# afanasyev-ilya/VectorGraphLibrary

Measured on AMD Instinct MI355X. Metric: TEPS (edges/s) BFS + SSSP on RMAT-24; value = direction-optimising BFS, sssp_value_teps = direction-optimising Bellman-Ford, higher is better.
Workload: dtype int32; 1 GPU; BFS direction-optimising on RMAT scale-24 (edge factor 32), 1xMI355X; vertices=16777216, edges=536870912, seed=1, parallelism=edge-cut x1, exchange_transport=none, vertex_numbering=degree-sorted (total)

## Files before the change

profiles/microbench/bfs_ab.py:

```python
#!/usr/bin/env python3
import argparse
import os
import sys
import time

sys.path.insert(0, os.path.dirname(os.path.dirname(os.path.dirname(os.path.abspath(__file__)))))
import torch

import bench
from vectorgraphlibrary_amd import api

ap = argparse.ArgumentParser()
ap.add_argument("--scale", type=int, default=24)
ap.add_argument("--steps", type=int, default=32)
ap.add_argument("--warmup", type=int, default=4)
ap.add_argument("--rounds", type=int, default=2)
ap.add_argument("--per-source", action="store_true")
ap.add_argument("variants", nargs="+")
args = ap.parse_args()

ctx = api.Context(0)
V = 1 << args.scale
src, dst = ctx.gen_rmat(args.scale, 32, 1)
g = api.Graph.from_coo(ctx, V, src, dst, with_incoming=True, renumber="total")
E = g.E
del src, dst
handles = {None: g}


def handle_for(heads):
    if heads not in handles:
        os.environ["VGL_BFS_HEADS"] = heads
        handles[heads] = api.Graph(ctx, V, g.out_rowptr, g.out_adj, g.in_rowptr, g.in_adj)
        print(f"handle for VGL_BFS_HEADS={heads}: {handles[heads].info()}", flush=True)
    return handles[heads]


sources = bench.pick_sources(g.out_rowptr, args.steps + args.warmup, 1)
ref = {}
for s in sources:
    lv, _ = api.bfs(g, s, api.BFS_TOP_DOWN, raw=True)
    ref[s] = lv.clone()
KERNELS = ("bfs_bottom_up", "bfs_bottom_up_heavy", "bfs_top_down", "bfs_small_levels", "bfs_bitmap_expand", "gnf")
variants = []
for v in args.variants:
    name, _, kv = v.partition(":")
    variants.append((name, dict(x.split("=", 1) for x in kv.split(",") if x)))
touched = set(k for _, env in variants for k in env)
results = {name: [] for name, _ in variants}
for rnd in range(args.rounds):
    for name, env in variants:
        for k in touched:
            os.environ.pop(k, None)
        os.environ.update(env)
        g = handle_for(env.get("VGL_BFS_HEADS"))
        bad = 0
        for s in sources[:args.warmup]:
            api.bfs(g, s, api.BFS_DIRECTION_OPT, raw=True)
        torch.cuda.synchronize()
        t0 = time.perf_counter()
        for s in sources[args.warmup:]:
            api.bfs(g, s, api.BFS_DIRECTION_OPT, raw=True)
        torch.cuda.synchronize()
        ms = (time.perf_counter() - t0) / args.steps * 1e3
        ctx.timing(True)
        stats = []
        prev = {k: 0.0 for k in KERNELS}
        for s in sources[args.warmup:]:
            lv, st = api.bfs(g, s, api.BFS_DIRECTION_OPT, raw=True)
            stats.append(st)
            bad += int(api.count_not_equal(ctx, lv, ref[s]) != 0)
            if args.per_source and rnd == 0:
                now = {k: ctx.timing_get(k)[1] for k in KERNELS}
                print(f"    {name} source {s}: td/bu {st['td_steps']}/{st['bu_steps']} td_edges {st['td_edges']} bu_probes {st['bu_edges']} bu_found {st['bu_found']} | "
                      + " ".join(f"{k.replace('bfs_', '')} {(now[k] - prev[k]) * 1e3:.0f}" for k in KERNELS if now[k] > prev[k]) + " us")
                prev = now
        torch.cuda.synchronize()
        kern = {k: ctx.timing_get(k) for k in KERNELS}
        ctx.timing(False)
# ... 6 lines not shown
```

vectorgraphlibrary_amd/csrc/bfs.hip:

```cpp
#include "vgl_hip_internal.h"
#include <chrono>
#include "vgl_gnf.h"
#include "vgl_blocked.h"

#ifndef VGL_BU_HEAVY_LANES
#define VGL_BU_HEAVY_LANES 16
#endif

__global__ __launch_bounds__(VGL_BLOCK) void vgl_k_bfs_init(int32_t V, int32_t source, int32_t *levels)
{
    for (int32_t v = blockIdx.x * VGL_BLOCK + threadIdx.x; v < V; v += gridDim.x * VGL_BLOCK)
        levels[v] = (v == source) ? 1 : -1;
}

__global__ __launch_bounds__(VGL_BLOCK) void vgl_k_bfs_init_all(int32_t fill, int32_t source, int32_t prev, int32_t *levels, int64_t words, uint64_t *visited,
                                                                uint64_t *front, uint64_t *next, uint32_t *tickets, unsigned long long *list_count)
{
    if (blockIdx.x == 0 && threadIdx.x == 0) {
        *list_count = 0ULL;
        if (prev >= fill) levels[prev] = -1;
        if (source >= fill) levels[source] = 1;
    }
    for (int32_t v = blockIdx.x * VGL_BLOCK + threadIdx.x; v < fill; v += gridDim.x * VGL_BLOCK)
        levels[v] = (v == source) ? 1 : -1;
    for (int64_t w = (int64_t)blockIdx.x * VGL_BLOCK + threadIdx.x; w < words; w += (int64_t)gridDim.x * VGL_BLOCK) {
        const uint64_t bit = (w == (source >> 6)) ? (1ULL << (source & 63)) : 0ULL;
        visited[w] = bit; front[w] = bit; next[w] = 0;
    }
    if (blockIdx.x == 0)
        for (int i = threadIdx.x; i < 4 * VGL_TICKET_WORDS; i += VGL_BLOCK) tickets[i] = 0;
}

__global__ __launch_bounds__(VGL_BLOCK) void vgl_k_tile_first(int32_t F, const int64_t *offs, int32_t *tile_first)
{
    for (int32_t p = blockIdx.x * VGL_BLOCK + threadIdx.x; p < F; p += gridDim.x * VGL_BLOCK) {
        const int64_t t0 = (offs[p] + VGL_TILE - 1) / VGL_TILE;
        const int64_t t1 = (offs[p + 1] + VGL_TILE - 1) / VGL_TILE;
        for (int64_t t = t0; t < t1; t++) tile_first[t] = p;
        if (offs[p] < offs[p + 1] && offs[p + 1] == offs[F]) tile_first[(offs[F] + VGL_TILE - 1) / VGL_TILE] = p;
    }
}

template <bool EMIT, bool COUNT, bool FILTER = true>
__global__ __launch_bounds__(VGL_BLOCK) void vgl_k_td_expand(const int32_t *ids, const int64_t *offs, const int32_t *tile_first,
                                                             int32_t F, int64_t M, const int64_t *rowptr, const int32_t *adj,
                                                             int32_t row_base, const uint64_t *visited, int32_t *levels,
                                                             int32_t next_level, uint64_t *next, int64_t *partials, uint32_t *ticket, int64_t *counters)
{
    __shared__ int s_map[VGL_TILE];
    __shared__ int64_t s_base[VGL_TILE];
    __shared__ int s_w[VGL_WAVES];
    const int64_t e0 = (int64_t)blockIdx.x * VGL_TILE;
    const int n = (int)min((int64_t)VGL_TILE, M - e0);
    const int p_first = tile_first[blockIdx.x];
    const int p_last = tile_first[blockIdx.x + 1];
    const int np = p_last - p_first + 1;
    const bool staged = np <= VGL_TILE;
    if (staged)
        for (int k = threadIdx.x; k < np; k += VGL_BLOCK) {
            const int p = p_first + k;
            s_base[k] = rowptr[ids[p] - row_base] - offs[p];
        }
// ... 22 lines not shown
#pragma unroll
        for (int j = 0; j < VGL_EPT; j++) unvis[j] = dsts[j] >= 0 && !((vw[j] >> (dsts[j] & 63)) & 1ULL);
    } else {
#pragma unroll
        for (int j = 0; j < VGL_EPT; j++) unvis[j] = dsts[j] >= 0;
    }
#else
#pragma unroll
    for (int j = 0; j < VGL_EPT; j++) unvis[j] = dsts[j] >= 0 && (!FILTER || !((visited[dsts[j] >> 6] >> (dsts[j] & 63)) & 1ULL));
#endif
#if VGL_TD_BATCH & 2
    int32_t lv[VGL_EPT];
#pragma unroll
    for (int j = 0; j < VGL_EPT; j++) lv[j] = levels[unvis[j] ? dsts[j] : 0];
#pragma unroll
    for (int j = 0; j < VGL_EPT; j++) fresh[j] = unvis[j] && lv[j] == -1;
#else
#pragma unroll
    for (int j = 0; j < VGL_EPT; j++) fresh[j] = unvis[j] && levels[dsts[j]] == -1;
#endif
    if (!COUNT) {
#pragma unroll
        for (int j = 0; j < VGL_EPT; j++)
            if (fresh[j]) {
                levels[dsts[j]] = next_level;
                if (EMIT) atomicOr((unsigned long long *)&next[dsts[j] >> 6], 1ULL << (dsts[j] & 63));
            }
        return;
    }
    __shared__ int64_t s64[VGL_WAVES];
    unsigned long long old[VGL_EPT];
#pragma unroll
    for (int j = 0; j < VGL_EPT; j++) {
        old[j] = ~0ULL;
// ... 206 lines not shown
        cpre += vgl_load_agent(vt_cnt + t);
        dpre += vgl_load_agent(vt_deg + t);
    }
    if (threadIdx.x == 0) {
        offs[ctot] = dtot;
        host[C_SKIPPED] = 0;
        vgl_publish2(counters, host, seq, C_FRONT, (int64_t)ctot, C_NEIGH, dtot);
    }
}
constexpr int VGL_SCAN_BLOCKS = 1024;
__device__ inline uint32_t vgl_match8(const int4 a, const int4 c, int32_t value)
{
    return (a.x == value) | ((a.y == value) << 1) | ((a.z == value) << 2) | ((a.w == value) << 3) |
           ((c.x == value) << 4) | ((c.y == value) << 5) | ((c.z == value) << 6) | ((c.w == value) << 7);
}
__global__ __launch_bounds__(VGL_BLOCK) void vgl_k_bfs_scan_bound(int32_t nrows, int32_t ntiles, int32_t row_base, const int32_t *levels, int32_t level,
                                                                 const int32_t *vt_min_deg, uint8_t *front_bytes, uint8_t *visited_bytes,
                                                                 int64_t *partials, uint32_t *ticket, int64_t *counters,
                                                                 volatile int64_t *host, int64_t seq, int32_t stale_front)
{
    __shared__ int64_t s64[VGL_WAVES];
    if (stale_front >= 0 && blockIdx.x == 0 && threadIdx.x == 0) front_bytes[stale_front >> 3] = 0;
    int64_t f = 0, m = 0;
    const int32_t stride = (int32_t)gridDim.x;
    int32_t t = (int32_t)blockIdx.x;
    for (; t + stride < ntiles && (t + stride + 1) * VGL_TILE <= nrows; t += 2 * stride) {
        const int32_t va = row_base + t * VGL_TILE + (int32_t)threadIdx.x * VGL_EPT, vb = va + stride * VGL_TILE;
        const int4 a0 = *reinterpret_cast<const int4 *>(levels + va), a1 = *reinterpret_cast<const int4 *>(levels + va + 4);
        const int4 b0 = *reinterpret_cast<const int4 *>(levels + vb), b1 = *reinterpret_cast<const int4 *>(levels + vb + 4);
        const uint32_t fa = vgl_match8(a0, a1, level), fb = vgl_match8(b0, b1, level);
        front_bytes[va >> 3] = (uint8_t)fa; visited_bytes[va >> 3] = (uint8_t)(0xFFu ^ vgl_match8(a0, a1, -1));
        front_bytes[vb >> 3] = (uint8_t)fb; visited_bytes[vb >> 3] = (uint8_t)(0xFFu ^ vgl_match8(b0, b1, -1));
        f += __popc(fa) + __popc(fb);
        m += (int64_t)__popc(fa) * vt_min_deg[t] + (int64_t)__popc(fb) * vt_min_deg[t + stride];
    }
    for (; t < ntiles; t += stride) {
        const int32_t r0 = t * VGL_TILE + (int32_t)threadIdx.x * VGL_EPT;
        if (r0 >= nrows) continue;
        const int32_t v0 = row_base + r0;
        uint32_t aux;
        const vgl_pred_equal_i32 pred{levels, level};
        const uint32_t bits = pred.bits8(v0, min(VGL_EPT, nrows - r0), &aux);
        front_bytes[v0 >> 3] = (uint8_t)bits;
        visited_bytes[v0 >> 3] = (uint8_t)aux;
        f += __popc(bits);
        m += (int64_t)__popc(bits) * vt_min_deg[t];
    }
    f = vgl_block_reduce_add(f, s64);
    m = vgl_block_reduce_add(m, s64);
    uint32_t dep = 0;
    if (threadIdx.x == 0) dep = vgl_put_agent(partials + 2 * blockIdx.x, f) ^ vgl_put_agent(partials + 2 * blockIdx.x + 1, m);
    if (!vgl_last_block(ticket, dep)) return;
    f = 0; m = 0;
    for (int b = threadIdx.x; b < (int)gridDim.x; b += VGL_BLOCK) { f += vgl_load_agent(partials + 2 * b); m += vgl_load_agent(partials + 2 * b + 1); }
    f = vgl_block_reduce_add(f, s64);
    m = vgl_block_reduce_add(m, s64);
// ... 622 lines not shown
    if (threadIdx.x == 0) { partials[blockIdx.x * 2] = cnt; partials[blockIdx.x * 2 + 1] = deg; }
}
__global__ __launch_bounds__(VGL_BLOCK) void vgl_k_apply_fold(int n, const int64_t *partials, int64_t *counters)
{
    __shared__ int64_t s64[VGL_WAVES];
    int64_t a = 0, b = 0;
    for (int i = threadIdx.x; i < n; i += VGL_BLOCK) { a += partials[i * 2]; b += partials[i * 2 + 1]; }
    a = vgl_block_reduce_add(a, s64);
    b = vgl_block_reduce_add(b, s64);
    if (threadIdx.x == 0) { counters[C_TMP0] = a; counters[C_TMP1] = b; }
}


template <bool EMIT, bool COUNT>
static void vgl_td_expand_launch(vgl_hip_ctx *c, vgl_hip_graph *g, int32_t F, int64_t M, const uint64_t *visited, int32_t *levels,
                                 int32_t next_level, uint64_t *next, bool filter = true)
{
    const auto kernel = filter ? vgl_k_td_expand<EMIT, COUNT, true> : vgl_k_td_expand<EMIT, COUNT, false>;
    hipLaunchKernelGGL(kernel, dim3((unsigned)vgl_ceil_div(M, VGL_TILE)), dim3(VGL_BLOCK), 0, c->stream, g->ids, g->offs, g->tile_first, F, M,
                       g->out.rowptr, g->out.adj, g->row_begin, visited, levels, next_level, next, COUNT ? g->bu_partials : (int64_t *)nullptr,
                       COUNT ? g->tickets + 3 * VGL_TICKET_WORDS : (uint32_t *)nullptr, COUNT ? c->d_counters : (int64_t *)nullptr);
}

constexpr int64_t VGL_TD_COUNT_TILES = 8192;
static int vgl_bfs_td_launch(vgl_hip_ctx *c, vgl_hip_graph *g, int32_t F, int64_t M, int32_t *levels, int32_t next_level, bool emit,
                             bool have_tile_first, bool count = false, bool filter = true)
{
    if (F <= 0 || M <= 0) return 0;
    if (!have_tile_first) hipLaunchKernelGGL(vgl_k_tile_first, dim3(vgl_grid(F, VGL_BLOCK, 8192)), dim3(VGL_BLOCK), 0, c->stream, F, g->offs, g->tile_first);
    {
        vgl_timed_launch tl(c, "bfs_top_down");
        if (emit && count) vgl_td_expand_launch<true, true>(c, g, F, M, g->bm_visited, levels, next_level, g->bm_next, filter);
        else if (emit) vgl_td_expand_launch<true, false>(c, g, F, M, g->bm_visited, levels, next_level, g->bm_next, filter);
        else vgl_td_expand_launch<false, false>(c, g, F, M, g->bm_visited, levels, next_level, g->bm_next, filter);
    }
    VGL_HIP_TRY(hipGetLastError());
    return 0;
}

int vgl_bfs_bm_gnf(vgl_hip_ctx *c, vgl_hip_graph *g, const uint64_t *front, bool count, bool write, int64_t M_known, bool advance, const vgl_do_hint *hint)
{
    const vgl_do_hint no_hint = {0, 0, 0, 0};
    const int64_t word0 = g->row_begin >> 6;
    const int64_t nwords = vgl_ceil_div(g->row_end, 64) - word0;
    const unsigned nb = (unsigned)vgl_ceil_div(nwords, VGL_BLOCK);
    if (count) {
        const int64_t seq = vgl_next_seq(c);
        {
            vgl_timed_launch tl(c, "gnf");
// ... 140 lines not shown

struct vgl_bfs_traversal {
    vgl_hip_ctx *c;
    vgl_hip_graph *g;
    int mode;
    int32_t *levels;
    vgl_bfs_params p;
    int32_t V;
    int64_t E, words, factor;
    unsigned bm_blocks;
    unsigned long long *list_count;
    std::chrono::steady_clock::time_point t0;

    int32_t source = -1;
    int32_t cur = 1;
    vgl_bfs_front front = vgl_bfs_front::bitmap;
    bool bottom_up = false;
    bool hint_ready = false, skipped = false, finished = false;
    int64_t F = 0, M = 0, prevF = 0, visited_total = 0;
    vgl_hip_bfs_stats st = {0, 0, 0, 0, 0, 0, 0, 0, 0, 0, 0};

    vgl_bfs_traversal(vgl_hip_ctx *c_, vgl_hip_graph *g_, int mode_, int32_t *levels_)
        : c(c_), g(g_), mode(mode_), levels(levels_), p(vgl_bfs_params_of(c_->bfs, g_->V, mode_)), V(g_->V), E(g_->out.edges)
    {
        words = vgl_ceil_div(V, 64);
        factor = vgl_do_factor(E, V);
        bm_blocks = (unsigned)vgl_ceil_div(words, VGL_BLOCK);
        list_count = reinterpret_cast<unsigned long long *>(c->d_counters + C_HEAVY);
    }

// ... 21 lines not shown
        const char *done = "count done (bitmap)";
        if (front != vgl_bfs_front::levels) {
            const bool advance = front == vgl_bfs_front::pending;
            const vgl_do_hint hint = {prevF, visited_total, (int64_t)V, factor};
            const bool hinted = hint_ready && advance && p.use_hints;
            VGL_TRY(vgl_bfs_bm_gnf(c, g, g->bm_front, true, false, -1, advance, hinted ? &hint : nullptr));
            skipped = hinted && c->h_counters[C_SKIPPED] != 0;
            front = skipped ? vgl_bfs_front::bitmap : vgl_bfs_front::counted_bitmap;
        } else if (p.scan_bound && g->nvtiles <= 8192) {
            const int64_t seq = vgl_next_seq(c);
            const int64_t scan_tiles = std::max<int64_t>(1, std::min<int64_t>(g->nvtiles, vgl_ceil_div(g->reach_rows, VGL_TILE)));
            const int32_t scan_rows = (int32_t)std::min<int64_t>(g->nrows, scan_tiles * VGL_TILE);
            {
                vgl_timed_launch tl(c, "gnf");
                hipLaunchKernelGGL(vgl_k_bfs_scan_bound, dim3((unsigned)std::min<int64_t>(scan_tiles, VGL_SCAN_BLOCKS)), dim3(VGL_BLOCK), 0, c->stream, scan_rows,
                                   (int32_t)scan_tiles, g->row_begin, (const int32_t *)levels, cur, (const int32_t *)g->vt_min_deg, (uint8_t *)g->bm_front.p,
                                   (uint8_t *)g->bm_visited.p, g->bu_partials, g->tickets + 0 * VGL_TICKET_WORDS, c->d_counters,
                                   (volatile int64_t *)c->h_counters, seq, source >= scan_rows ? source : -1);
            }
            VGL_HIP_TRY(hipGetLastError());
            VGL_TRY(vgl_wait_counters(c, seq));
            front = vgl_bfs_front::bitmap;
            const int64_t f = c->h_counters[C_FRONT], m_lb = c->h_counters[C_NEIGH];
            if (vgl_do_turn_bottom_up(f, m_lb, prevF, visited_total + f, V, factor)) {
                F = f; M = m_lb; skipped = true; hint_ready = false;
                trace("count done (levels scan)");
                return 0;
            }
            VGL_TRY(vgl_bfs_bm_gnf(c, g, g->bm_front, true, false, -1, false, nullptr));
            front = vgl_bfs_front::counted_bitmap;
        } else {
            vgl_pred_equal_i32 pred{levels, cur};
            VGL_TRY(vgl_gnf_run(c, g, pred, g->ids, g->offs, (uint8_t *)g->bm_front.p, (uint8_t *)g->bm_visited.p, nullptr, false, true));
            front = vgl_bfs_front::counted_scan;
            done = "count done (levels scan)";
        }
        F = c->h_counters[C_FRONT]; M = c->h_counters[C_NEIGH];
        hint_ready = false;
        trace(done);
        return 0;
    }

    int small_levels(int32_t listF, int32_t src, bool from_bitmap)
    {
        if (from_bitmap) {
            vgl_timed_launch tl(c, "bfs_bitmap_expand");
            hipLaunchKernelGGL(vgl_k_bm_expand, dim3(bm_blocks), dim3(VGL_BLOCK), 0, c->stream, words, g->bm_front, g->out.rowptr, g->out.adj, g->bm_visited,
                               g->bm_next, levels, cur + 1, g->ids, list_count, (int32_t)VGL_SMALL_F, g->bu_partials);
        }
        const int64_t seq = vgl_next_seq(c);
        {
            vgl_timed_launch tl(c, "bfs_small_levels");
            hipLaunchKernelGGL(vgl_k_bfs_small_levels, dim3(1), dim3(VGL_SMALL_THREADS), 0, c->stream, g->ids, listF, src, g->out.rowptr, g->out.adj,
                               g->bm_visited, g->bm_next, levels, from_bitmap ? cur + 1 : cur, p.small_m, c->d_counters, (volatile int64_t *)c->h_counters,
                               seq, from_bitmap ? list_count : (unsigned long long *)nullptr, (const int64_t *)g->bu_partials, from_bitmap ? (int)bm_blocks : 0,
                               g->bm_front, g->offs, g->tile_first);
        }
        VGL_HIP_TRY(hipGetLastError());
        VGL_TRY(vgl_wait_counters(c, seq));
        return 0;
    }
    void book_small(int64_t firstF)
    {
        const int64_t *h = c->h_counters;
        const int64_t run = h[C_TMP0], later = h[C_TMP1];
        st.td_steps += (int32_t)run; st.edges_examined += h[C_EDGES]; st.td_edges += h[C_EDGES];
        st.td_frontier += firstF + later;
        visited_total += later; st.levels += (int32_t)(run - 1); st.frontier_total += later;
        if (run > 1) prevF = h[C_JUMP];
// ... 10 lines not shown
        const int64_t m_level = c->h_counters[C_CHANGED], n_next = c->h_counters[C_BU_FOUND];
        book_top_down(F, m_level);
        prevF = F;
        cur++;
        if (n_next == 0) { finished = true; return 0; }
        if (c->h_counters[C_TMP0] > 0) {
            begin_level(n_next);
            prevF = n_next;
            book_small(n_next);
        } else front = vgl_bfs_front::pending;
        return 0;
    }
    int blocked_level()
    {
        trace("counted -> blocked level");
        VGL_TRY(vgl_bfs_blocked_level(c, g, levels, cur + 1));
        trace("blocked level done");
        front = vgl_bfs_front::pending;
        book_top_down(F, M);
        cur++;
        return 0;
    }
    int top_down_level()
    {
        switch (front) {
        case vgl_bfs_front::ids: break;
        case vgl_bfs_front::counted_bitmap: VGL_TRY(vgl_bfs_bm_gnf(c, g, g->bm_front, false, true, M)); break;
        case vgl_bfs_front::counted_scan: {
            vgl_pred_equal_i32 pred{levels, cur};
            vgl_timed_launch tl(c, "gnf");
            hipLaunchKernelGGL(vgl_k_gnf_write<vgl_pred_equal_i32>, dim3((unsigned)g->nvtiles), dim3(VGL_BLOCK), 0, c->stream, pred,
                               g->nrows, g->row_begin, g->out.rowptr, g->vt_cnt_off, g->vt_deg_off, g->ids, g->offs, (int32_t *)nullptr, (int64_t)0);
            break;
        }
        default: VGL_FAIL("bfs_run: internal error (frontier not counted)");
        }
        trace("ids written");
        const bool have_tile_first = front != vgl_bfs_front::counted_scan;
        if (p.small_m > 0 && have_tile_first && F <= VGL_SMALL_F && M <= p.small_m) {
            trace("counted + ids -> list kernel");
            VGL_TRY(small_levels((int32_t)F, -1, false));
            trace("list kernel done");
            book_small(F);
            return 0;
        }
        const bool is_late = late();
        const bool emit = M <= p.td_emit_edges || is_late;
        const bool td_counts = emit && p.use_hints && vgl_ceil_div(M, VGL_TILE) <= VGL_TD_COUNT_TILES;
        const bool filter = is_late || (double)visited_total >= p.td_filter_share * (double)V;
        trace(emit ? "counted + ids -> top-down (emitting)" : "counted + ids -> top-down (levels only)");
        VGL_TRY(vgl_bfs_td_launch(c, g, (int32_t)F, M, levels, cur + 1, emit, have_tile_first, td_counts, filter));
        trace("top-down done");
        hint_ready = td_counts && F > 0 && M > 0;
        front = emit ? vgl_bfs_front::pending : vgl_bfs_front::levels;
        book_top_down(F, M);
        cur++;
        return 0;
    }
    int bottom_up_level()
    {
        if (front == vgl_bfs_front::levels || front == vgl_bfs_front::pending) VGL_FAIL("bfs_run: internal error (bitmaps missing)");
        int64_t seq = 0;
        trace("-> bottom-up");
        const bool filtered = F <= p.filter_f;
        if (filtered) trace("bottom-up through the folded frontier");
        VGL_TRY(vgl_bfs_bu_launch(c, g, levels, cur + 1, g->bm_visited, g->bm_front, g->bm_next, &seq, filtered));
        hipLaunchKernelGGL(vgl_k_bm_advance, dim3(vgl_grid(words, VGL_BLOCK, 8192)), dim3(VGL_BLOCK), 0, c->stream, words, g->bm_visited, g->bm_front, g->bm_next);
        VGL_HIP_TRY(hipGetLastError());
        VGL_TRY(vgl_wait_counters(c, seq));
        st.bu_steps++; st.edges_examined += c->h_counters[C_BU_EDGES];
        st.bu_edges += c->h_counters[C_BU_EDGES]; st.bu_found += c->h_counters[C_BU_FOUND];
        F = c->h_counters[C_BU_FOUND]; M = 0;
        front = vgl_bfs_front::bitmap;
        cur++;
        return 0;
    }

    int run(int32_t source_, int32_t prev = -1)
    {
        source = source_;
        const int32_t fill = prev >= 0 ? g->reach_rows : V;
        hipLaunchKernelGGL(vgl_k_bfs_init_all, dim3(vgl_grid(std::max<int64_t>(fill, words), VGL_BLOCK, 8192)), dim3(VGL_BLOCK), 0, c->stream, fill, source, prev,
                           levels, words, g->bm_visited, g->bm_front, g->bm_next, g->tickets, list_count);
        t0 = std::chrono::steady_clock::now();
        if (p.small_m > 0) {
            VGL_TRY(small_levels(1, source, false));
            if (c->h_counters[C_TMP0] > 0) {
                begin_level(1);
                prevF = 1;
                book_small(1);
            }
        }
        while (!finished) {
            if (front != vgl_bfs_front::ids && !bottom_up) VGL_TRY(count());
            if (F == 0) break;
            begin_level(F);
            if (mode == VGL_HIP_BFS_DIRECTION_OPT) {
                if (!bottom_up) bottom_up = vgl_do_turn_bottom_up(F, M, prevF, visited_total, V, factor);
// ... 35 lines not shown
    spec.gather_rows = 1;
    spec.skip_self = 1;
    spec.value_bits = 1;
    return vgl_blocked_build(c, g->out, g->nrows, g->row_begin, g->V, spec, &g->blk_bfs);
}

int vgl_hip_bfs_init(vgl_hip_ctx *c, int32_t V, int32_t source, int32_t *d_levels)
{
    if (!c || !d_levels) VGL_FAIL("bfs_init: null argument");
    if (source < 0 || source >= V) VGL_FAIL("bfs_init: source vertex out of range");
    hipLaunchKernelGGL(vgl_k_bfs_init, dim3(vgl_grid(V, VGL_BLOCK, 8192)), dim3(VGL_BLOCK), 0, c->stream, V, source, d_levels);
    VGL_HIP_TRY(hipGetLastError());
    return 0;
}

static int vgl_bfs_run_from(vgl_hip_ctx *c, vgl_hip_graph *g, int32_t source, int32_t prev, int mode, int32_t *d_levels, vgl_hip_bfs_stats *stats)
{
    if (!c || !g || !d_levels) VGL_FAIL("bfs_run: null argument");
    if (g->row_begin != 0 || g->row_end != g->V) VGL_FAIL("bfs_run: graph handle must own all rows (use the step API for shards)");
    if (mode != VGL_HIP_BFS_TOP_DOWN && mode != VGL_HIP_BFS_DIRECTION_OPT) VGL_FAIL("bfs_run: unknown mode");
    if (mode == VGL_HIP_BFS_DIRECTION_OPT && !g->in.rowptr) VGL_FAIL("bfs_run: direction-optimising mode needs the incoming CSR");
    if (source < 0 || source >= g->V) VGL_FAIL("bfs_run: source vertex out of range");
    vgl_ctx_refresh_env(c);
    vgl_bfs_traversal t(c, g, mode, d_levels);
    VGL_TRY(t.run(source, prev));
    if (stats) *stats = t.st;
    return 0;
}

int vgl_hip_bfs_run(vgl_hip_ctx *c, vgl_hip_graph *g, int32_t source, int mode, int32_t *d_levels, vgl_hip_bfs_stats *stats)
{
    return vgl_bfs_run_from(c, g, source, -1, mode, d_levels, stats);
}

int vgl_hip_bfs_run_batch(vgl_hip_ctx *c, vgl_hip_graph *g, const int32_t *sources, int32_t count, int mode, int32_t *d_levels, vgl_hip_bfs_stats *stats)
{
    if (!sources || count < 0) VGL_FAIL("bfs_run_batch: null argument");
    for (int32_t i = 0; i < count; i++)
        VGL_TRY(vgl_bfs_run_from(c, g, sources[i], i > 0 ? sources[i - 1] : -1, mode, d_levels, stats ? stats + i : nullptr));
    return 0;
}

int vgl_hip_bfs_step_top_down(vgl_hip_ctx *c, vgl_hip_graph *g, int32_t *d_levels, int32_t level, const uint64_t *d_visited_bits,
                              int64_t *local_frontier, int64_t *local_edges)
{
    if (!c || !g || !d_levels) VGL_FAIL("bfs_step_top_down: null argument");
    const uint64_t *visited = d_visited_bits;
    if (!visited) {
        hipLaunchKernelGGL(vgl_k_levels_to_bitmap<true>, dim3(vgl_grid(g->V, VGL_BLOCK, 8192)), dim3(VGL_BLOCK), 0, c->stream, g->V, d_levels, -1,
                           g->bm_visited);
        visited = g->bm_visited;
    }
    vgl_pred_equal_i32 pred{d_levels, level};
    VGL_TRY(vgl_gnf_run(c, g, pred, g->ids, g->offs, nullptr, nullptr, nullptr, true, true));
    const int64_t F = c->h_counters[C_FRONT], M = c->h_counters[C_NEIGH];
    if (local_frontier) *local_frontier = F;
    if (local_edges) *local_edges = M;
    if (F > 0 && M > 0) {
        hipLaunchKernelGGL(vgl_k_tile_first, dim3(vgl_grid(F, VGL_BLOCK, 8192)), dim3(VGL_BLOCK), 0, c->stream, (int32_t)F, g->offs, g->tile_first);
        vgl_timed_launch tl(c, "bfs_top_down");
        vgl_td_expand_launch<false, false>(c, g, (int32_t)F, M, visited, d_levels, level + 1, nullptr);
    }
    VGL_HIP_TRY(hipGetLastError());
    return 0;
}

int vgl_hip_bfs_step_top_down_bits(vgl_hip_ctx *c, vgl_hip_graph *g, int32_t *d_levels, int32_t level, const uint64_t *d_visited_bits,
                                   const uint64_t *d_front_bits, uint64_t *d_next_bits, int64_t *local_frontier, int64_t *local_edges)
{
    if (!c || !g || !d_levels || !d_visited_bits || !d_front_bits || !d_next_bits) VGL_FAIL("bfs_step_top_down_bits: null argument");
    if (g->row_begin & 63) VGL_FAIL("bfs_step_top_down_bits: the first owned row must be a multiple of 64");
    VGL_TRY(vgl_bfs_bm_gnf(c, g, d_front_bits, true, true));
    const int64_t F = c->h_counters[C_FRONT], M = c->h_counters[C_NEIGH];
    if (local_frontier) *local_frontier = F;
    if (local_edges) *local_edges = M;
    const int64_t emit_edges = c->bfs.shard_td_emit_edges >= 0 ? c->bfs.shard_td_emit_edges : vgl_bfs_td_emit_edges(g->V);
    const bool emit = M <= emit_edges;
    const int64_t words = vgl_ceil_div(g->V, 64);
    if (emit) VGL_TRY(vgl_zero_words(c, d_next_bits, words));
    if (F > 0 && M > 0) {
        vgl_timed_launch tl(c, "bfs_top_down");
        if (emit) vgl_td_expand_launch<true, false>(c, g, (int32_t)F, M, d_visited_bits, d_levels, level + 1, d_next_bits);
        else vgl_td_expand_launch<false, false>(c, g, (int32_t)F, M, d_visited_bits, d_levels, level + 1, d_next_bits);
    }
    if (!emit) {
        vgl_timed_launch tl(c, "gnf");
        hipLaunchKernelGGL(vgl_k_levels_to_bitmap<false>, dim3(vgl_grid(g->V, VGL_BLOCK, 8192)), dim3(VGL_BLOCK), 0, c->stream, g->V, (const int32_t *)d_levels, level + 1, d_next_bits);
    }
    VGL_HIP_TRY(hipGetLastError());
    return 0;
}

int vgl_hip_bfs_step_bottom_up(vgl_hip_ctx *c, vgl_hip_graph *g, int32_t *d_levels, int32_t level, const uint64_t *d_visited_bits,
                               const uint64_t *d_front_bits, uint64_t *d_next_bits, int64_t *found, int64_t *probed)
{
    if (!c || !g || !d_levels || !d_visited_bits || !d_front_bits || !d_next_bits) VGL_FAIL("bfs_step_bottom_up: null argument");
    if (!g->in.rowptr) VGL_FAIL("bfs_step_bottom_up: the incoming CSR of the owned rows is required");
    VGL_TRY(vgl_zero_words(c, d_next_bits, vgl_ceil_div(g->V, 64)));
// ... 105 lines not shown
```

vectorgraphlibrary_amd/csrc/context.hip:

```cpp
#include "vgl_hip_internal.h"
#include <unordered_set>
#include <cstdio>
#include <cstring>
#include <mutex>
#include <algorithm>

static thread_local std::string g_last_error;

int vgl_set_error(const char *file, int line, const char *msg)
{
    char buf[512];
    const char *base = strrchr(file, '/');
    snprintf(buf, sizeof(buf), "vgl_hip: %s (%s:%d)", msg, base ? base + 1 : file, line);
    g_last_error = buf;
    return 1;
}

static hipMemPool_t g_lib_pool[64];
static bool g_lib_pool_tried[64];
static std::mutex g_lib_pool_mutex;
hipMemPool_t vgl_lib_pool(int device)
{
    if (device < 0 || device >= 64) return nullptr;
    std::lock_guard<std::mutex> lock(g_lib_pool_mutex);
// ... 43 lines not shown
        for (char **e = environ; *e; e++)
            if (strncmp(*e, "VGL_", 4) == 0)
                if (const char *eq = strchr(*e, '=')) c->env[std::string(*e, (size_t)(eq - *e))] = std::string(eq + 1);
    vgl_bfs_tunables t;
    auto str = [&](const char *n) -> const char * { auto it = c->env.find(n); return it == c->env.end() ? nullptr : it->second.c_str(); };
    auto on = [&](const char *n) { const char *v = str(n); return v && v[0] == '1'; };
    if (const char *v = str("VGL_TD_EMIT_EDGES")) t.td_emit_edges = atoll(v);
    if (const char *v = str("VGL_BFS_SMALL_M")) t.small_m = atoll(v);
    if (const char *v = str("VGL_BFS_BM_EXPAND")) t.bm_expand = atoll(v);
    if (const char *v = str("VGL_BFS_FILTER_F")) t.filter_f = atoll(v);
    if (const char *v = str("VGL_SHARD_TD_EMIT_EDGES")) t.shard_td_emit_edges = atoll(v);
    if (const char *v = str("VGL_TD_FILTER_SHARE")) t.td_filter_share = atof(v);
    if (const char *v = str("VGL_TD_LATE_SHARE")) t.td_late_share = atof(v);
    if (const char *v = str("VGL_BFS_BLOCKED_SHARE")) t.blocked_share = atof(v);
    if (const char *v = str("VGL_SHARD_SPARSE_CAP")) t.shard_sparse_cap = std::max(0, atoi(v));
    t.no_hint = on("VGL_BFS_NO_HINT"); t.no_scan_bound = on("VGL_BFS_NO_SCAN_BOUND"); t.trace = on("VGL_BFS_TRACE");
    c->bfs = t;
}
const char *vgl_env(vgl_hip_ctx *c, const char *name)
{
    vgl_ctx_refresh_env(c);
    auto it = c->env.find(name);
    return it == c->env.end() ? nullptr : it->second.c_str();
}
int64_t vgl_env_int(vgl_hip_ctx *c, const char *name, int64_t dflt, int64_t lo, int64_t hi)
{
    const char *s = vgl_env(c, name);
    const int64_t v = (s && *s) ? strtoll(s, nullptr, 10) : dflt;
    return std::min(hi, std::max(lo, v));
}

// ... 243 lines not shown
```

vectorgraphlibrary_amd/csrc/vgl_gnf.h:

```cpp
#pragma once
#include "vgl_hip_internal.h"

#ifdef __HIPCC__

struct vgl_pred_equal_i32 {
    const int32_t *values; int32_t value;
    __device__ uint32_t bits8(int32_t v0, int nvalid, uint32_t *aux) const
    {
        uint32_t b = 0, n = 0;
        if (nvalid == 8) {
            const int4 a = *reinterpret_cast<const int4 *>(values + v0);
            const int4 c = *reinterpret_cast<const int4 *>(values + v0 + 4);
            b = (a.x == value) | ((a.y == value) << 1) | ((a.z == value) << 2) | ((a.w == value) << 3) |
                ((c.x == value) << 4) | ((c.y == value) << 5) | ((c.z == value) << 6) | ((c.w == value) << 7);
            n = (a.x != -1) | ((a.y != -1) << 1) | ((a.z != -1) << 2) | ((a.w != -1) << 3) |
                ((c.x != -1) << 4) | ((c.y != -1) << 5) | ((c.z != -1) << 6) | ((c.w != -1) << 7);
        } else {
            for (int j = 0; j < nvalid; j++) {
                const int32_t x = values[v0 + j];
                b |= (uint32_t)(x == value) << j;
                n |= (uint32_t)(x != -1) << j;
            }
        }
        *aux = n;
        return b;
    }
};
struct vgl_pred_nonzero_i32 {
    const int32_t *flags;
    __device__ uint32_t bits8(int32_t v0, int nvalid, uint32_t *aux) const
    {
        uint32_t b = 0;
        *aux = 0;
        if (nvalid == 8) {
            const int4 a = *reinterpret_cast<const int4 *>(flags + v0);
            const int4 c = *reinterpret_cast<const int4 *>(flags + v0 + 4);
            b = (a.x != 0) | ((a.y != 0) << 1) | ((a.z != 0) << 2) | ((a.w != 0) << 3) |
                ((c.x != 0) << 4) | ((c.y != 0) << 5) | ((c.z != 0) << 6) | ((c.w != 0) << 7);
        } else {
            for (int j = 0; j < nvalid; j++) b |= (uint32_t)(flags[v0 + j] != 0) << j;
        }
        return b;
// ... 272 lines not shown
```

vectorgraphlibrary_amd/csrc/vgl_hip_internal.h:

```cpp
#pragma once
#include <hip/hip_runtime.h>
#include <stdint.h>
#include <string>
#include <map>
#include <memory>
#include <vector>
#include "../../include/vgl_hip.h"

constexpr int VGL_BLOCK = 256;
constexpr int VGL_EPT = 8;
constexpr int VGL_TILE = VGL_BLOCK * VGL_EPT;
constexpr int VGL_WAVES = VGL_BLOCK / 64;
constexpr int VGL_FOLD_WORDS = 2048;

int vgl_set_error(const char *file, int line, const char *msg);
#define VGL_FAIL(msg) return vgl_set_error(__FILE__, __LINE__, (msg))
#define VGL_HIP_TRY(expr)                                                          \
    do {                                                                           \
        hipError_t _e = (expr);                                                    \
        if (_e != hipSuccess) return vgl_set_error(__FILE__, __LINE__, hipGetErrorString(_e)); \
    } while (0)
#define VGL_TRY(expr)            \
    do {                         \
        int _s = (expr);         \
// ... 8 lines not shown
    C_NSLOTS = 32
};
constexpr int VGL_NSHARD = 1024;

struct vgl_timing_slot {
    int64_t launches = 0;
    std::vector<std::pair<hipEvent_t, hipEvent_t>> pending;
    double total_ms = 0.0;
};

struct vgl_bfs_tunables {
    int64_t td_emit_edges = -1, small_m = -1, bm_expand = -1, shard_td_emit_edges = -1, filter_f = -1;
    double td_filter_share = -1.0, td_late_share = -1.0, blocked_share = -1.0;
    int shard_sparse_cap = -1;
    bool no_hint = false, no_scan_bound = false, trace = false;
};

struct vgl_hip_ctx {
    std::map<std::string, std::string> env;
    uint64_t env_signature = 0;
    vgl_bfs_tunables bfs;
    int device = 0;
    hipStream_t stream = nullptr;
    bool own_stream = false;
    int64_t *d_counters = nullptr;
    int64_t *d_shards = nullptr;
    int64_t *h_counters = nullptr;
    int64_t publish_seq = 0;
    double *d_partials = nullptr;
    size_t partials_cap = 0;
// ... 410 lines not shown
```

Before: 1933 billion edges/s.

## Use per-traversal level offsets in batched BFS to skip level-array refills

Batched BFS no longer clears the levels array between sources. Each traversal writes levels shifted by a running offset, and every kernel treats values at or below the offset floor as unvisited: top-down expand, the scan-bound count, the new level predicate and the init kernel. A full refill still runs on the first and last source, or when the offset nears INT32 overflow. This removes most per-source O(reach_rows) init traffic, at the cost of an extra compare parameter threaded through many kernels and intermediate level arrays that are not directly meaningful.

```diff
diff --git a/profiles/microbench/bfs_ab.py b/profiles/microbench/bfs_ab.py
--- a/profiles/microbench/bfs_ab.py
+++ b/profiles/microbench/bfs_ab.py
@@ -16,6 +16,7 @@
 ap.add_argument("--warmup", type=int, default=4)
 ap.add_argument("--rounds", type=int, default=2)
 ap.add_argument("--per-source", action="store_true")
+ap.add_argument("--batch", action="store_true")
 ap.add_argument("variants", nargs="+")
 args = ap.parse_args()
 
@@ -41,6 +42,7 @@
 for s in sources:
     lv, _ = api.bfs(g, s, api.BFS_TOP_DOWN, raw=True)
     ref[s] = lv.clone()
+lv_buf = ctx.empty(V, torch.int32)
 KERNELS = ("bfs_bottom_up", "bfs_bottom_up_heavy", "bfs_top_down", "bfs_small_levels", "bfs_bitmap_expand", "gnf")
 variants = []
 for v in args.variants:
@@ -59,10 +61,15 @@
             api.bfs(g, s, api.BFS_DIRECTION_OPT, raw=True)
         torch.cuda.synchronize()
         t0 = time.perf_counter()
-        for s in sources[args.warmup:]:
-            api.bfs(g, s, api.BFS_DIRECTION_OPT, raw=True)
+        if args.batch:
+            lv_batch, _ = api.bfs_batch(g, sources[args.warmup:], api.BFS_DIRECTION_OPT, levels=lv_buf)
+        else:
+            for s in sources[args.warmup:]:
+                api.bfs(g, s, api.BFS_DIRECTION_OPT, raw=True)
         torch.cuda.synchronize()
         ms = (time.perf_counter() - t0) / args.steps * 1e3
+        if args.batch:
+            bad += int(api.count_not_equal(ctx, lv_batch, ref[sources[-1]]) != 0)
         ctx.timing(True)
         stats = []
         prev = {k: 0.0 for k in KERNELS}
diff --git a/vectorgraphlibrary_amd/csrc/bfs.hip b/vectorgraphlibrary_amd/csrc/bfs.hip
--- a/vectorgraphlibrary_amd/csrc/bfs.hip
+++ b/vectorgraphlibrary_amd/csrc/bfs.hip
@@ -13,16 +13,17 @@
         levels[v] = (v == source) ? 1 : -1;
 }
 
-__global__ __launch_bounds__(VGL_BLOCK) void vgl_k_bfs_init_all(int32_t fill, int32_t source, int32_t prev, int32_t *levels, int64_t words, uint64_t *visited,
-                                                                uint64_t *front, uint64_t *next, uint32_t *tickets, unsigned long long *list_count)
+__global__ __launch_bounds__(VGL_BLOCK) void vgl_k_bfs_init_all(int32_t fill, int32_t source, int32_t first, int32_t reset, int32_t *levels, int64_t words,
+                                                                uint64_t *visited, uint64_t *front, uint64_t *next, uint32_t *tickets,
+                                                                unsigned long long *list_count)
 {
     if (blockIdx.x == 0 && threadIdx.x == 0) {
         *list_count = 0ULL;
-        if (prev >= fill) levels[prev] = -1;
-        if (source >= fill) levels[source] = 1;
+        if (reset >= fill) levels[reset] = -1;
+        if (source >= fill) levels[source] = first;
     }
     for (int32_t v = blockIdx.x * VGL_BLOCK + threadIdx.x; v < fill; v += gridDim.x * VGL_BLOCK)
-        levels[v] = (v == source) ? 1 : -1;
+        levels[v] = (v == source) ? first : -1;
     for (int64_t w = (int64_t)blockIdx.x * VGL_BLOCK + threadIdx.x; w < words; w += (int64_t)gridDim.x * VGL_BLOCK) {
         const uint64_t bit = (w == (source >> 6)) ? (1ULL << (source & 63)) : 0ULL;
         visited[w] = bit; front[w] = bit; next[w] = 0;
@@ -45,7 +46,8 @@
 __global__ __launch_bounds__(VGL_BLOCK) void vgl_k_td_expand(const int32_t *ids, const int64_t *offs, const int32_t *tile_first,
                                                              int32_t F, int64_t M, const int64_t *rowptr, const int32_t *adj,
                                                              int32_t row_base, const uint64_t *visited, int32_t *levels,
-                                                             int32_t next_level, uint64_t *next, int64_t *partials, uint32_t *ticket, int64_t *counters)
+                                                             int32_t next_level, int32_t floor, uint64_t *next, int64_t *partials, uint32_t *ticket,
+                                                             int64_t *counters)
 {
     __shared__ int s_map[VGL_TILE];
     __shared__ int64_t s_base[VGL_TILE];
@@ -98,10 +100,10 @@
 #pragma unroll
     for (int j = 0; j < VGL_EPT; j++) lv[j] = levels[unvis[j] ? dsts[j] : 0];
 #pragma unroll
-    for (int j = 0; j < VGL_EPT; j++) fresh[j] = unvis[j] && lv[j] == -1;
+    for (int j = 0; j < VGL_EPT; j++) fresh[j] = unvis[j] && lv[j] <= floor;
 #else
 #pragma unroll
-    for (int j = 0; j < VGL_EPT; j++) fresh[j] = unvis[j] && levels[dsts[j]] == -1;
+    for (int j = 0; j < VGL_EPT; j++) fresh[j] = unvis[j] && levels[dsts[j]] <= floor;
 #endif
     if (!COUNT) {
 #pragma unroll
@@ -338,10 +340,15 @@
     return (a.x == value) | ((a.y == value) << 1) | ((a.z == value) << 2) | ((a.w == value) << 3) |
            ((c.x == value) << 4) | ((c.y == value) << 5) | ((c.z == value) << 6) | ((c.w == value) << 7);
 }
+__device__ inline uint32_t vgl_above8(const int4 a, const int4 c, int32_t floor)
+{
+    return (a.x > floor) | ((a.y > floor) << 1) | ((a.z > floor) << 2) | ((a.w > floor) << 3) |
+           ((c.x > floor) << 4) | ((c.y > floor) << 5) | ((c.z > floor) << 6) | ((c.w > floor) << 7);
+}
 __global__ __launch_bounds__(VGL_BLOCK) void vgl_k_bfs_scan_bound(int32_t nrows, int32_t ntiles, int32_t row_base, const int32_t *levels, int32_t level,
                                                                  const int32_t *vt_min_deg, uint8_t *front_bytes, uint8_t *visited_bytes,
                                                                  int64_t *partials, uint32_t *ticket, int64_t *counters,
-                                                                 volatile int64_t *host, int64_t seq, int32_t stale_front)
+                                                                 volatile int64_t *host, int64_t seq, int32_t stale_front, int32_t floor)
 {
     __shared__ int64_t s64[VGL_WAVES];
     if (stale_front >= 0 && blockIdx.x == 0 && threadIdx.x == 0) front_bytes[stale_front >> 3] = 0;
@@ -353,8 +360,8 @@
         const int4 a0 = *reinterpret_cast<const int4 *>(levels + va), a1 = *reinterpret_cast<const int4 *>(levels + va + 4);
         const int4 b0 = *reinterpret_cast<const int4 *>(levels + vb), b1 = *reinterpret_cast<const int4 *>(levels + vb + 4);
         const uint32_t fa = vgl_match8(a0, a1, level), fb = vgl_match8(b0, b1, level);
-        front_bytes[va >> 3] = (uint8_t)fa; visited_bytes[va >> 3] = (uint8_t)(0xFFu ^ vgl_match8(a0, a1, -1));
-        front_bytes[vb >> 3] = (uint8_t)fb; visited_bytes[vb >> 3] = (uint8_t)(0xFFu ^ vgl_match8(b0, b1, -1));
+        front_bytes[va >> 3] = (uint8_t)fa; visited_bytes[va >> 3] = (uint8_t)vgl_above8(a0, a1, floor);
+        front_bytes[vb >> 3] = (uint8_t)fb; visited_bytes[vb >> 3] = (uint8_t)vgl_above8(b0, b1, floor);
         f += __popc(fa) + __popc(fb);
         m += (int64_t)__popc(fa) * vt_min_deg[t] + (int64_t)__popc(fb) * vt_min_deg[t + stride];
     }
@@ -363,7 +370,7 @@
         if (r0 >= nrows) continue;
         const int32_t v0 = row_base + r0;
         uint32_t aux;
-        const vgl_pred_equal_i32 pred{levels, level};
+        const vgl_pred_level_i32 pred{levels, level, floor};
         const uint32_t bits = pred.bits8(v0, min(VGL_EPT, nrows - r0), &aux);
         front_bytes[v0 >> 3] = (uint8_t)bits;
         visited_bytes[v0 >> 3] = (uint8_t)aux;
@@ -1016,25 +1023,25 @@
 
 template <bool EMIT, bool COUNT>
 static void vgl_td_expand_launch(vgl_hip_ctx *c, vgl_hip_graph *g, int32_t F, int64_t M, const uint64_t *visited, int32_t *levels,
-                                 int32_t next_level, uint64_t *next, bool filter = true)
+                                 int32_t next_level, int32_t floor, uint64_t *next, bool filter = true)
 {
     const auto kernel = filter ? vgl_k_td_expand<EMIT, COUNT, true> : vgl_k_td_expand<EMIT, COUNT, false>;
     hipLaunchKernelGGL(kernel, dim3((unsigned)vgl_ceil_div(M, VGL_TILE)), dim3(VGL_BLOCK), 0, c->stream, g->ids, g->offs, g->tile_first, F, M,
-                       g->out.rowptr, g->out.adj, g->row_begin, visited, levels, next_level, next, COUNT ? g->bu_partials : (int64_t *)nullptr,
+                       g->out.rowptr, g->out.adj, g->row_begin, visited, levels, next_level, floor, next, COUNT ? g->bu_partials : (int64_t *)nullptr,
                        COUNT ? g->tickets + 3 * VGL_TICKET_WORDS : (uint32_t *)nullptr, COUNT ? c->d_counters : (int64_t *)nullptr);
 }
 
 constexpr int64_t VGL_TD_COUNT_TILES = 8192;
-static int vgl_bfs_td_launch(vgl_hip_ctx *c, vgl_hip_graph *g, int32_t F, int64_t M, int32_t *levels, int32_t next_level, bool emit,
+static int vgl_bfs_td_launch(vgl_hip_ctx *c, vgl_hip_graph *g, int32_t F, int64_t M, int32_t *levels, int32_t next_level, int32_t floor, bool emit,
                              bool have_tile_first, bool count = false, bool filter = true)
 {
     if (F <= 0 || M <= 0) return 0;
     if (!have_tile_first) hipLaunchKernelGGL(vgl_k_tile_first, dim3(vgl_grid(F, VGL_BLOCK, 8192)), dim3(VGL_BLOCK), 0, c->stream, F, g->offs, g->tile_first);
     {
         vgl_timed_launch tl(c, "bfs_top_down");
-        if (emit && count) vgl_td_expand_launch<true, true>(c, g, F, M, g->bm_visited, levels, next_level, g->bm_next, filter);
-        else if (emit) vgl_td_expand_launch<true, false>(c, g, F, M, g->bm_visited, levels, next_level, g->bm_next, filter);
-        else vgl_td_expand_launch<false, false>(c, g, F, M, g->bm_visited, levels, next_level, g->bm_next, filter);
+        if (emit && count) vgl_td_expand_launch<true, true>(c, g, F, M, g->bm_visited, levels, next_level, floor, g->bm_next, filter);
+        else if (emit) vgl_td_expand_launch<true, false>(c, g, F, M, g->bm_visited, levels, next_level, floor, g->bm_next, filter);
+        else vgl_td_expand_launch<false, false>(c, g, F, M, g->bm_visited, levels, next_level, floor, g->bm_next, filter);
     }
     VGL_HIP_TRY(hipGetLastError());
     return 0;
@@ -1205,6 +1212,7 @@
 
     int32_t source = -1;
     int32_t cur = 1;
+    int32_t off = 0;
     vgl_bfs_front front = vgl_bfs_front::bitmap;
     bool bottom_up = false;
     bool hint_ready = false, skipped = false, finished = false;
@@ -1256,9 +1264,9 @@
             {
                 vgl_timed_launch tl(c, "gnf");
                 hipLaunchKernelGGL(vgl_k_bfs_scan_bound, dim3((unsigned)std::min<int64_t>(scan_tiles, VGL_SCAN_BLOCKS)), dim3(VGL_BLOCK), 0, c->stream, scan_rows,
-                                   (int32_t)scan_tiles, g->row_begin, (const int32_t *)levels, cur, (const int32_t *)g->vt_min_deg, (uint8_t *)g->bm_front.p,
+                                   (int32_t)scan_tiles, g->row_begin, (const int32_t *)levels, off + cur, (const int32_t *)g->vt_min_deg, (uint8_t *)g->bm_front.p,
                                    (uint8_t *)g->bm_visited.p, g->bu_partials, g->tickets + 0 * VGL_TICKET_WORDS, c->d_counters,
-                                   (volatile int64_t *)c->h_counters, seq, source >= scan_rows ? source : -1);
+                                   (volatile int64_t *)c->h_counters, seq, source >= scan_rows ? source : -1, off);
             }
             VGL_HIP_TRY(hipGetLastError());
             VGL_TRY(vgl_wait_counters(c, seq));
@@ -1272,7 +1280,7 @@
             VGL_TRY(vgl_bfs_bm_gnf(c, g, g->bm_front, true, false, -1, false, nullptr));
             front = vgl_bfs_front::counted_bitmap;
         } else {
-            vgl_pred_equal_i32 pred{levels, cur};
+            vgl_pred_level_i32 pred{levels, off + cur, off};
             VGL_TRY(vgl_gnf_run(c, g, pred, g->ids, g->offs, (uint8_t *)g->bm_front.p, (uint8_t *)g->bm_visited.p, nullptr, false, true));
             front = vgl_bfs_front::counted_scan;
             done = "count done (levels scan)";
@@ -1288,13 +1296,13 @@
         if (from_bitmap) {
             vgl_timed_launch tl(c, "bfs_bitmap_expand");
             hipLaunchKernelGGL(vgl_k_bm_expand, dim3(bm_blocks), dim3(VGL_BLOCK), 0, c->stream, words, g->bm_front, g->out.rowptr, g->out.adj, g->bm_visited,
-                               g->bm_next, levels, cur + 1, g->ids, list_count, (int32_t)VGL_SMALL_F, g->bu_partials);
+                               g->bm_next, levels, off + cur + 1, g->ids, list_count, (int32_t)VGL_SMALL_F, g->bu_partials);
         }
         const int64_t seq = vgl_next_seq(c);
         {
             vgl_timed_launch tl(c, "bfs_small_levels");
             hipLaunchKernelGGL(vgl_k_bfs_small_levels, dim3(1), dim3(VGL_SMALL_THREADS), 0, c->stream, g->ids, listF, src, g->out.rowptr, g->out.adj,
-                               g->bm_visited, g->bm_next, levels, from_bitmap ? cur + 1 : cur, p.small_m, c->d_counters, (volatile int64_t *)c->h_counters,
+                               g->bm_visited, g->bm_next, levels, off + (from_bitmap ? cur + 1 : cur), p.small_m, c->d_counters, (volatile int64_t *)c->h_counters,
                                seq, from_bitmap ? list_count : (unsigned long long *)nullptr, (const int64_t *)g->bu_partials, from_bitmap ? (int)bm_blocks : 0,
                                g->bm_front, g->offs, g->tile_first);
         }
@@ -1335,7 +1343,7 @@
     int blocked_level()
     {
         trace("counted -> blocked level");
-        VGL_TRY(vgl_bfs_blocked_level(c, g, levels, cur + 1));
+        VGL_TRY(vgl_bfs_blocked_level(c, g, levels, off + cur + 1));
         trace("blocked level done");
         front = vgl_bfs_front::pending;
         book_top_down(F, M);
@@ -1348,9 +1356,9 @@
         case vgl_bfs_front::ids: break;
         case vgl_bfs_front::counted_bitmap: VGL_TRY(vgl_bfs_bm_gnf(c, g, g->bm_front, false, true, M)); break;
         case vgl_bfs_front::counted_scan: {
-            vgl_pred_equal_i32 pred{levels, cur};
+            vgl_pred_level_i32 pred{levels, off + cur, off};
             vgl_timed_launch tl(c, "gnf");
-            hipLaunchKernelGGL(vgl_k_gnf_write<vgl_pred_equal_i32>, dim3((unsigned)g->nvtiles), dim3(VGL_BLOCK), 0, c->stream, pred,
+            hipLaunchKernelGGL(vgl_k_gnf_write<vgl_pred_level_i32>, dim3((unsigned)g->nvtiles), dim3(VGL_BLOCK), 0, c->stream, pred,
                                g->nrows, g->row_begin, g->out.rowptr, g->vt_cnt_off, g->vt_deg_off, g->ids, g->offs, (int32_t *)nullptr, (int64_t)0);
             break;
         }
@@ -1370,7 +1378,7 @@
         const bool td_counts = emit && p.use_hints && vgl_ceil_div(M, VGL_TILE) <= VGL_TD_COUNT_TILES;
         const bool filter = is_late || (double)visited_total >= p.td_filter_share * (double)V;
         trace(emit ? "counted + ids -> top-down (emitting)" : "counted + ids -> top-down (levels only)");
-        VGL_TRY(vgl_bfs_td_launch(c, g, (int32_t)F, M, levels, cur + 1, emit, have_tile_first, td_counts, filter));
+        VGL_TRY(vgl_bfs_td_launch(c, g, (int32_t)F, M, levels, off + cur + 1, off, emit, have_tile_first, td_counts, filter));
         trace("top-down done");
         hint_ready = td_counts && F > 0 && M > 0;
         front = emit ? vgl_bfs_front::pending : vgl_bfs_front::levels;
@@ -1385,7 +1393,7 @@
         trace("-> bottom-up");
         const bool filtered = F <= p.filter_f;
         if (filtered) trace("bottom-up through the folded frontier");
-        VGL_TRY(vgl_bfs_bu_launch(c, g, levels, cur + 1, g->bm_visited, g->bm_front, g->bm_next, &seq, filtered));
+        VGL_TRY(vgl_bfs_bu_launch(c, g, levels, off + cur + 1, g->bm_visited, g->bm_front, g->bm_next, &seq, filtered));
         hipLaunchKernelGGL(vgl_k_bm_advance, dim3(vgl_grid(words, VGL_BLOCK, 8192)), dim3(VGL_BLOCK), 0, c->stream, words, g->bm_visited, g->bm_front, g->bm_next);
         VGL_HIP_TRY(hipGetLastError());
         VGL_TRY(vgl_wait_counters(c, seq));
@@ -1397,12 +1405,14 @@
         return 0;
     }
 
-    int run(int32_t source_, int32_t prev = -1)
+    int run(int32_t source_, int32_t prev = -1, bool refill = true, int32_t off_ = 0)
     {
         source = source_;
-        const int32_t fill = prev >= 0 ? g->reach_rows : V;
-        hipLaunchKernelGGL(vgl_k_bfs_init_all, dim3(vgl_grid(std::max<int64_t>(fill, words), VGL_BLOCK, 8192)), dim3(VGL_BLOCK), 0, c->stream, fill, source, prev,
-                           levels, words, g->bm_visited, g->bm_front, g->bm_next, g->tickets, list_count);
+        off = off_;
+        const int32_t fill = prev < 0 ? V : refill ? g->reach_rows : 0;
+        const int32_t reset = prev >= g->reach_rows ? prev : -1;
+        hipLaunchKernelGGL(vgl_k_bfs_init_all, dim3(vgl_grid(std::max<int64_t>(fill, words), VGL_BLOCK, 8192)), dim3(VGL_BLOCK), 0, c->stream, fill, source, off + 1,
+                           reset, levels, words, g->bm_visited, g->bm_front, g->bm_next, g->tickets, list_count);
         t0 = std::chrono::steady_clock::now();
         if (p.small_m > 0) {
             VGL_TRY(small_levels(1, source, false));
@@ -1468,30 +1478,42 @@
     return 0;
 }
 
-static int vgl_bfs_run_from(vgl_hip_ctx *c, vgl_hip_graph *g, int32_t source, int32_t prev, int mode, int32_t *d_levels, vgl_hip_bfs_stats *stats)
+static int vgl_bfs_run_from(vgl_hip_ctx *c, vgl_hip_graph *g, int32_t source, int32_t prev, bool refill, int32_t off, int mode, int32_t *d_levels,
+                            vgl_hip_bfs_stats *stats)
 {
     if (!c || !g || !d_levels) VGL_FAIL("bfs_run: null argument");
     if (g->row_begin != 0 || g->row_end != g->V) VGL_FAIL("bfs_run: graph handle must own all rows (use the step API for shards)");
     if (mode != VGL_HIP_BFS_TOP_DOWN && mode != VGL_HIP_BFS_DIRECTION_OPT) VGL_FAIL("bfs_run: unknown mode");
     if (mode == VGL_HIP_BFS_DIRECTION_OPT && !g->in.rowptr) VGL_FAIL("bfs_run: direction-optimising mode needs the incoming CSR");
     if (source < 0 || source >= g->V) VGL_FAIL("bfs_run: source vertex out of range");
-    vgl_ctx_refresh_env(c);
     vgl_bfs_traversal t(c, g, mode, d_levels);
-    VGL_TRY(t.run(source, prev));
+    VGL_TRY(t.run(source, prev, refill, off));
     if (stats) *stats = t.st;
     return 0;
 }
 
 int vgl_hip_bfs_run(vgl_hip_ctx *c, vgl_hip_graph *g, int32_t source, int mode, int32_t *d_levels, vgl_hip_bfs_stats *stats)
 {
-    return vgl_bfs_run_from(c, g, source, -1, mode, d_levels, stats);
+    if (c) vgl_ctx_refresh_env(c);
+    return vgl_bfs_run_from(c, g, source, -1, true, 0, mode, d_levels, stats);
 }
 
 int vgl_hip_bfs_run_batch(vgl_hip_ctx *c, vgl_hip_graph *g, const int32_t *sources, int32_t count, int mode, int32_t *d_levels, vgl_hip_bfs_stats *stats)
 {
     if (!sources || count < 0) VGL_FAIL("bfs_run_batch: null argument");
-    for (int32_t i = 0; i < count; i++)
-        VGL_TRY(vgl_bfs_run_from(c, g, sources[i], i > 0 ? sources[i - 1] : -1, mode, d_levels, stats ? stats + i : nullptr));
+    if (c) vgl_ctx_refresh_env(c);
+    const bool offsets = c && g && !c->bfs.batch_refill;
+    int64_t limit = offsets ? (int64_t)INT32_MAX - g->V - 2 : 0;
+    if (offsets && c->bfs.offset_limit >= 0) limit = std::min(limit, c->bfs.offset_limit);
+    int64_t off = 0;
+    for (int32_t i = 0; i < count; i++) {
+        const bool refill = i == 0 || i == count - 1 || !offsets || off > limit;
+        if (refill) off = 0;
+        vgl_hip_bfs_stats st;
+        VGL_TRY(vgl_bfs_run_from(c, g, sources[i], i > 0 ? sources[i - 1] : -1, refill, (int32_t)off, mode, d_levels, &st));
+        if (stats) stats[i] = st;
+        off += st.levels;
+    }
     return 0;
 }
 
@@ -1513,7 +1535,7 @@
     if (F > 0 && M > 0) {
         hipLaunchKernelGGL(vgl_k_tile_first, dim3(vgl_grid(F, VGL_BLOCK, 8192)), dim3(VGL_BLOCK), 0, c->stream, (int32_t)F, g->offs, g->tile_first);
         vgl_timed_launch tl(c, "bfs_top_down");
-        vgl_td_expand_launch<false, false>(c, g, (int32_t)F, M, visited, d_levels, level + 1, nullptr);
+        vgl_td_expand_launch<false, false>(c, g, (int32_t)F, M, visited, d_levels, level + 1, 0, nullptr);
     }
     VGL_HIP_TRY(hipGetLastError());
     return 0;
@@ -1534,8 +1556,8 @@
     if (emit) VGL_TRY(vgl_zero_words(c, d_next_bits, words));
     if (F > 0 && M > 0) {
         vgl_timed_launch tl(c, "bfs_top_down");
-        if (emit) vgl_td_expand_launch<true, false>(c, g, (int32_t)F, M, d_visited_bits, d_levels, level + 1, d_next_bits);
-        else vgl_td_expand_launch<false, false>(c, g, (int32_t)F, M, d_visited_bits, d_levels, level + 1, d_next_bits);
+        if (emit) vgl_td_expand_launch<true, false>(c, g, (int32_t)F, M, d_visited_bits, d_levels, level + 1, 0, d_next_bits);
+        else vgl_td_expand_launch<false, false>(c, g, (int32_t)F, M, d_visited_bits, d_levels, level + 1, 0, d_next_bits);
     }
     if (!emit) {
         vgl_timed_launch tl(c, "gnf");
diff --git a/vectorgraphlibrary_amd/csrc/context.hip b/vectorgraphlibrary_amd/csrc/context.hip
--- a/vectorgraphlibrary_amd/csrc/context.hip
+++ b/vectorgraphlibrary_amd/csrc/context.hip
@@ -81,7 +81,9 @@
     if (const char *v = str("VGL_TD_LATE_SHARE")) t.td_late_share = atof(v);
     if (const char *v = str("VGL_BFS_BLOCKED_SHARE")) t.blocked_share = atof(v);
     if (const char *v = str("VGL_SHARD_SPARSE_CAP")) t.shard_sparse_cap = std::max(0, atoi(v));
+    if (const char *v = str("VGL_BFS_OFFSET_LIMIT")) t.offset_limit = atoll(v);
     t.no_hint = on("VGL_BFS_NO_HINT"); t.no_scan_bound = on("VGL_BFS_NO_SCAN_BOUND"); t.trace = on("VGL_BFS_TRACE");
+    t.batch_refill = on("VGL_BFS_BATCH_REFILL");
     c->bfs = t;
 }
 const char *vgl_env(vgl_hip_ctx *c, const char *name)
diff --git a/vectorgraphlibrary_amd/csrc/vgl_gnf.h b/vectorgraphlibrary_amd/csrc/vgl_gnf.h
--- a/vectorgraphlibrary_amd/csrc/vgl_gnf.h
+++ b/vectorgraphlibrary_amd/csrc/vgl_gnf.h
@@ -26,6 +26,29 @@
         return b;
     }
 };
+struct vgl_pred_level_i32 {
+    const int32_t *values; int32_t value, floor;
+    __device__ uint32_t bits8(int32_t v0, int nvalid, uint32_t *aux) const
+    {
+        uint32_t b = 0, n = 0;
+        if (nvalid == 8) {
+            const int4 a = *reinterpret_cast<const int4 *>(values + v0);
+            const int4 c = *reinterpret_cast<const int4 *>(values + v0 + 4);
+            b = (a.x == value) | ((a.y == value) << 1) | ((a.z == value) << 2) | ((a.w == value) << 3) |
+                ((c.x == value) << 4) | ((c.y == value) << 5) | ((c.z == value) << 6) | ((c.w == value) << 7);
+            n = (a.x > floor) | ((a.y > floor) << 1) | ((a.z > floor) << 2) | ((a.w > floor) << 3) |
+                ((c.x > floor) << 4) | ((c.y > floor) << 5) | ((c.z > floor) << 6) | ((c.w > floor) << 7);
+        } else {
+            for (int j = 0; j < nvalid; j++) {
+                const int32_t x = values[v0 + j];
+                b |= (uint32_t)(x == value) << j;
+                n |= (uint32_t)(x > floor) << j;
+            }
+        }
+        *aux = n;
+        return b;
+    }
+};
 struct vgl_pred_nonzero_i32 {
     const int32_t *flags;
     __device__ uint32_t bits8(int32_t v0, int nvalid, uint32_t *aux) const
diff --git a/vectorgraphlibrary_amd/csrc/vgl_hip_internal.h b/vectorgraphlibrary_amd/csrc/vgl_hip_internal.h
--- a/vectorgraphlibrary_amd/csrc/vgl_hip_internal.h
+++ b/vectorgraphlibrary_amd/csrc/vgl_hip_internal.h
@@ -46,6 +46,8 @@
     double td_filter_share = -1.0, td_late_share = -1.0, blocked_share = -1.0;
     int shard_sparse_cap = -1;
     bool no_hint = false, no_scan_bound = false, trace = false;
+    bool batch_refill = false;
+    int64_t offset_limit = -1;
 };
 
 struct vgl_hip_ctx {
```

Result: faster. 1973 billion edges/s (median of 6 runs) (+2.1%).
